# ska-telescope/ska-sdp-continuum-imaging-pipeline

Measured on AMD Instinct MI355X. Metric: Mvis/s gridded (invert) on 8k^2 grid, support=8, higher is better.
Workload: dtype f64; 1 GPU; C3: 390,625 rows x 256 ch = 100,000,000 vis/GPU -> 8192x8192 grid (4096^2 image), support 8, 2-D, fp64 accumulate; input=Stokes-I visibilities + effective weights (cip_ms2dirty), rows_per_gpu=390625, channels=256, grid=8192, image=4096, support=8, wstacking=False, parallelism=single GPU

## Files before the change

### ska-sdp-continuum-imaging-pipeline_amd/csrc/cip_grid.hip

```cpp
#include <type_traits>

#include "cip_internal.h"

namespace cip {


__global__ __launch_bounds__(1024) void prep_final_kernel(const double* partial, int nblocks, double* out2) {
  double sum[4] = {0.0, 0.0, 0.0, 0.0}, mx = 0.0;
  for (int i0 = threadIdx.x; i0 < nblocks; i0 += 4 * 1024) {
    if (i0 + 3 * 1024 < nblocks) {
      double2 p[4];
#pragma unroll
      for (int k = 0; k < 4; ++k) p[k] = reinterpret_cast<const double2*>(partial)[i0 + k * 1024];
#pragma unroll
      for (int k = 0; k < 4; ++k) {
        sum[k] += p[k].x;
        mx = fmax(mx, p[k].y);
      }
      continue;
    }
#pragma unroll
    for (int k = 0; k < 4; ++k) {
      const int i = i0 + k * 1024;
      if (i < nblocks) {
        const double2 p = reinterpret_cast<const double2*>(partial)[i];
        sum[k] += p.x;
        mx = fmax(mx, p.y);
      }
    }
  }
  double s = (sum[0] + sum[1]) + (sum[2] + sum[3]);
  for (int d = 32; d > 0; d >>= 1) {
    s += __shfl_xor(s, d, 64);
    mx = fmax(mx, __shfl_xor(mx, d, 64));
  }
  __shared__ double ss[16], sm[16];
  if ((threadIdx.x & 63) == 0) {
    ss[threadIdx.x >> 6] = s;
    sm[threadIdx.x >> 6] = mx;
  }
  __syncthreads();
  if (threadIdx.x == 0) {
    double t = 0.0, m = 0.0;
    for (int w = 0; w < 16; ++w) {
      t += ss[w];
      m = fmax(m, sm[w]);
    }
    out2[0] = t;
    out2[1] = m;
  }
}

hipError_t launch_prep_final(const double* partial, int nblocks, double* out2, hipStream_t s) {
  prep_final_kernel<<<dim3(1), dim3(1024), 0, s>>>(partial, nblocks, out2);
  return hipGetLastError();
}

__global__ void add_scalar_kernel(const double* src, double* dst) {
  if (threadIdx.x == 0) *dst += *src;
}

hipError_t launch_add_scalar(const double* src, double* dst, hipStream_t s) {
  add_scalar_kernel<<<dim3(1), dim3(64), 0, s>>>(src, dst);
  return hipGetLastError();
}

constexpr int kOrderThreads = 256;
constexpr int kOrderPer = kOrderWindow / kOrderThreads;
constexpr int kOrderBatch = kOrderThreads * kOrderPer;
static_assert(kOrderBatch == kOrderWindow, "one order block per window");

template <int WIDE, bool PH, int NC = 16>
__global__ __launch_bounds__(kOrderThreads, 8) void order_kernel(const uint8_t* __restrict__ vis_class, RowMap m,
                                                                 const uint64_t* __restrict__ runs,
                                                                 const int64_t* __restrict__ run_goff,
                                                                 const Chunk* __restrict__ windows,
                                                                 void* __restrict__ perm, int dP) {
  __shared__ __attribute__((aligned(16))) unsigned s_cnt[32];
  __shared__ unsigned s_keep[PH ? NC : 1], s_eff[PH ? NC : 1];
  __shared__ union {
    struct {
      uint64_t rec[kOrderBatch];
      int64_t delta[WIDE == 1 ? kOrderBatch : 1];
      int off[kOrderBatch + 1];
      uint16_t idx[kOrderBatch];
    } a;
    struct {
      unsigned S[kOrderBatch], M[kOrderBatch];
    } b;
  } sh;
  uint64_t* const s_rec = sh.a.rec;
  int* const s_off = sh.a.off;
  uint16_t* const s_idx = sh.a.idx;
  unsigned* const s_S = sh.b.S;
  unsigned* const s_M = sh.b.M;
  const Chunk ch = windows[blockIdx.x];
  const int64_t sb = ch.g0;
  const int nsb = (int)(ch.g1 - ch.g0);
  const int nst = (int)(ch.last_run - ch.first_run + 1);
  for (int k = threadIdx.x; k < nst; k += kOrderThreads) {
    s_off[k] = (int)(run_goff[ch.first_run + k] - sb);
    const uint64_t rec = runs[ch.first_run + k];
    if constexpr (WIDE == 2) {
      if (m.pk_runs) {
        s_rec[k] = rec;
      } else {
        const int64_t row = (int64_t)(rec >> 32), c = (int64_t)((rec >> 16) & 0xffff);
// ... 301 lines not shown
```

### ska-sdp-continuum-imaging-pipeline_amd/csrc/cip_internal.h

```cpp
#pragma once
#include <hip/hip_runtime.h>
#include <stdint.h>

#include <string>

#include "cip.h"
#include "cip_common.h"

namespace cip {

int set_error(int code, const std::string& msg);
#define CIP_HIP_CHECK(expr)                                                     \
  do {                                                                          \
    hipError_t e_ = (expr);                                                     \
    if (e_ != hipSuccess)                                                       \
      return ::cip::set_error(CIP_EHIP, std::string(#expr) + ": " +            \
                                            hipGetErrorString(e_));            \
  } while (0)

bool place_rows64();
bool order_classes32();

int64_t scan_tmp_elems(int64_t n);
hipError_t scan_run_offsets(const uint64_t* runs, int64_t nruns, int64_t* run_goff, int64_t* tmp,
                            const uint32_t* run_keys, hipStream_t s);
hipError_t exclusive_scan_i64(int64_t* data, int64_t n, int64_t* tmp, hipStream_t s);

hipError_t launch_freq_scale(const double* freq, int64_t nchan, double* fx, unsigned* err, hipStream_t s);
hipError_t launch_w_range(const double* uvw, int64_t nrow, double fxmin, double fxmax, double* partial,
                          int nblocks, hipStream_t s);
int plan_place_blocks(int64_t nvis);
hipError_t launch_prep_reduce(const RowMap& m, const void* vis, int vis_dtype, const void* wgt, int wgt_dtype,
                              const GridGeometry& g, unsigned* err_flag, double* partial, hipStream_t s);
hipError_t launch_plan_place(const double* uvw, const double* fx, const RowMap& m,
                             const void* vis, int vis_dtype, const void* wgt, int wgt_dtype, const GridGeometry& g,
                             unsigned* err_flag, uint8_t* vis_class, int64_t* blk_cnt, uint32_t* park_key,
                             uint64_t* park_run, double* partial, int64_t* hist0, hipStream_t s);
hipError_t launch_ragged_lengths(const int32_t* c0, const int32_t* c1, int64_t nrow, int64_t nchan, int64_t* out,
                                 unsigned* err, hipStream_t s);
hipError_t launch_ragged_expand(const int64_t* off, const int32_t* c0, int64_t nrow, int64_t* delta,
                                uint32_t* seg_row, hipStream_t s);
int64_t radix_blocks(int64_t n);
hipError_t launch_radix_hist(const uint32_t* keys, int64_t n, const int64_t* blk_cnt, int64_t nsub, int G, int shift,
                             int64_t* hist, hipStream_t s);
hipError_t launch_radix_group_hist(const int64_t* hist0, int64_t nsub, int G, int64_t* hg, hipStream_t s);
hipError_t launch_radix_scatter(const uint32_t* keys, const uint64_t* vals, int64_t n, const int64_t* blk_cnt,
                                int64_t nsub, int G, int shift, const int64_t* hist, uint32_t* keys_out,
                                uint64_t* vals_out, hipStream_t s);
hipError_t launch_tile_offsets(const uint32_t* keys, int64_t nruns, int64_t ntiles, int64_t* tile_run_off,
                               uint32_t kmask, hipStream_t s);
hipError_t launch_dirty_mask(const int64_t* tile_vis, const GridGeometry& g, uint8_t* mask, uint32_t* bits,
                             hipStream_t s);
hipError_t launch_tile_vis(const int64_t* run_goff, const int64_t* tile_run_off, int64_t ntiles,
                           int64_t* tile_vis_off, int64_t* tile_vis, hipStream_t s);
hipError_t launch_chunk_counts(const int64_t* tile_vis, int64_t ntiles, int64_t chunk_vis, int full_first,
                               int64_t* out, hipStream_t s);
hipError_t launch_chunk_emit(const int64_t* tile_vis_off, const int64_t* tile_vis, const int64_t* chunk_off,
                             const int64_t* run_goff, const int64_t* tile_run_off, int64_t ntiles,
                             int64_t chunk_vis, int full_first, int64_t nchunks, Chunk* chunks, hipStream_t s);
hipError_t launch_plane_chunk_counts(const int64_t* tile_vis_off, int64_t ntxy, int64_t ntw, int64_t ngroups,
                                     int group, int support, int64_t cv, int64_t* out, hipStream_t s);
hipError_t launch_plane_chunk_emit(const int64_t* tile_vis_off, const int64_t* chunk_off, const int64_t* run_goff,
                                   const int64_t* tile_run_off, int64_t ntxy, int64_t ntw, int64_t ngroups,
                                   int group, int support, int64_t cv, int64_t nchunks, Chunk* chunks, hipStream_t s);
hipError_t launch_gather_i64(const int64_t* src, int64_t stride, int64_t count, int64_t* dst,
                             hipStream_t s);

hipError_t launch_add_scalar(const double* src, double* dst, hipStream_t s);
hipError_t launch_prep_final(const double* partial, int nblocks, double* out2, hipStream_t s);
struct PlanView {
  const double *uvw = nullptr, *fx = nullptr;
  const void *vis = nullptr, *wgt = nullptr;
  RowMap m;
  const uint64_t* runs = nullptr;
  const int64_t *run_goff = nullptr, *tile_run_off = nullptr;
  const void* perm = nullptr;
  const Chunk* chunks = nullptr;
};
struct ScatterLaunch {
  PlanView plan;
  int64_t chunk_begin = 0, nchunks = 0;
  GridGeometry g;
  int64_t plane = 0;
  double fixed_scale = 1.0;
  double* grid = nullptr;
  int support = 0, vis_dtype = CIP_C64, wgt_dtype = CIP_NONE;
  bool packed = false;
  int group = 1;
  bool share_cus = false, store_private = false;
};
template <int W>
hipError_t launch_scatter_w(const ScatterLaunch& a, dim3 gd, unsigned lds_extra, hipStream_t s);
template <int W>
hipError_t launch_scatter_large_w(const ScatterLaunch& a, dim3 gd, hipStream_t s);
hipError_t launch_scatter(const ScatterLaunch& a, hipStream_t s);
hipError_t launch_order(const uint8_t* vis_class, const RowMap& m, const uint64_t* runs, const int64_t* run_goff,
                        const Chunk* windows, int64_t nwindows, void* perm, int phase_support, hipStream_t s);
bool order_phases_ok(const RowMap& m, int support);
hipError_t launch_crop_correct_2d(const double* grid, const GridGeometry& g, int64_t npix_x, int64_t npix_y,
                                  const double* cx, const double* cy, double* dirty, hipStream_t s);
hipError_t launch_wplane_accumulate(const double* grid, const GridGeometry& g, int64_t npix_x, int64_t npix_y,
                                    double pixsize_x, double pixsize_y, double w_plane, int first,
                                    double* acc, hipStream_t s);
hipError_t launch_wfinal_correct(double* acc, int64_t npix_x, int64_t npix_y, double pixsize_x, double pixsize_y,
                                 const double* cx, const double* cy, const double* fw_table, int64_t fw_n,
                                 double fw_dnu, double dw, int64_t i0, int64_t nrows, const double* norm,
                                 const float* acc_f32, hipStream_t s);

struct DegridOut {
  void* vis_io;
  int vis_dtype;
  const void* wgt;
  int wgt_dtype;
  int subtract;
  double2* acc;
};
struct DegridLaunch {
  PlanView plan;
  int64_t chunk_begin = 0, nchunks = 0;
  GridGeometry g;
  int64_t plane = 0;
  const double* planes = nullptr;
// ... 75 lines not shown
```

### ska-sdp-continuum-imaging-pipeline_amd/csrc/cip_plan.hip

```cpp
#include <type_traits>

#include "cip_internal.h"

namespace cip {

constexpr int kScanThreads = 1024;
constexpr int kScanItems = 4;
constexpr int64_t kScanBlock = (int64_t)kScanThreads * kScanItems;

template <int RUNS>
__device__ __forceinline__ int64_t run_length_at(const void* __restrict__ src, int64_t k) {
  if constexpr (RUNS == 2) {
    return (int64_t)(((const uint32_t*)src)[k] >> kRunLenShift) + 1;
  } else {
    const uint64_t rec = ((const uint64_t*)src)[k];
    return (int64_t)(rec & 0xffff) - (int64_t)((rec >> 16) & 0xffff);
  }
}
template <int RUNS>
__global__ __launch_bounds__(kScanThreads) void scan_local_kernel(int64_t* data, int64_t n, int64_t* block_sums,
                                                                  const void* __restrict__ runs) {
  __shared__ int64_t wave_tot[kScanThreads / 64];
  const int64_t base = (int64_t)blockIdx.x * kScanBlock + (int64_t)threadIdx.x * kScanItems;
  int64_t v[kScanItems];
  int64_t tsum = 0;
  if (base + kScanItems <= (RUNS ? n - 1 : n)) {
#pragma unroll
    for (int i = 0; i < kScanItems; ++i) {
      if constexpr (RUNS) {
        v[i] = run_length_at<RUNS>(runs, base + i);
      } else {
        v[i] = data[base + i];
      }
    }
  } else {
#pragma unroll
    for (int i = 0; i < kScanItems; ++i) {
      if constexpr (RUNS) {
        v[i] = 0;
        if (base + i < n - 1) v[i] = run_length_at<RUNS>(runs, base + i);
      } else {
        v[i] = (base + i < n) ? data[base + i] : 0;
      }
    }
  }
#pragma unroll
  for (int i = 0; i < kScanItems; ++i) tsum += v[i];
  const int lane = threadIdx.x & 63, wave = threadIdx.x >> 6;
  int64_t incl = tsum;
#pragma unroll
  for (int d = 1; d < 64; d <<= 1) {
    int64_t o = __shfl_up(incl, d, 64);
    if (lane >= d) incl += o;
  }
  if (lane == 63) wave_tot[wave] = incl;
  __syncthreads();
  if (wave == 0) {
    int64_t t = (lane < kScanThreads / 64) ? wave_tot[lane] : 0;
#pragma unroll
    for (int d = 1; d < 64; d <<= 1) {
      int64_t o = __shfl_up(t, d, 64);
      if (lane >= d) t += o;
    }
    if (lane < kScanThreads / 64) wave_tot[lane] = t;
  }
  __syncthreads();
  int64_t run = incl - tsum + (wave > 0 ? wave_tot[wave - 1] : 0);
#pragma unroll
  for (int i = 0; i < kScanItems; ++i) {
    if (base + i < n) data[base + i] = run;
    run += v[i];
  }
  if (threadIdx.x == kScanThreads - 1) block_sums[blockIdx.x] = run;
}

__global__ void scan_add_kernel(int64_t* data, int64_t n, const int64_t* offsets) {
  const int64_t i = (int64_t)blockIdx.x * kScanBlock + threadIdx.x;
  const int64_t off = offsets[blockIdx.x];
  if (i + (int64_t)(kScanItems - 1) * kScanThreads < n) {
    int64_t v[kScanItems];
#pragma unroll
    for (int k = 0; k < kScanItems; ++k) v[k] = data[i + (int64_t)k * kScanThreads];
#pragma unroll
    for (int k = 0; k < kScanItems; ++k) data[i + (int64_t)k * kScanThreads] = v[k] + off;
    return;
  }
#pragma unroll
  for (int k = 0; k < kScanItems; ++k) {
    const int64_t j = i + (int64_t)k * kScanThreads;
    if (j < n) data[j] += off;
  }
}

int64_t scan_tmp_elems(int64_t n) {
  int64_t total = 0;
  while (n > 1) {
    const int64_t nb = (n + kScanBlock - 1) / kScanBlock;
    total += nb;
    n = nb;
  }
  return total + 1;
}

struct ScanLengths {
  int kind;
  const void* src;
};
static hipError_t scan_impl(int64_t* data, int64_t n, int64_t* tmp, ScanLengths from, hipStream_t s) {
  if (n <= 0) return hipSuccess;
  const int64_t nb = (n + kScanBlock - 1) / kScanBlock;
  hipError_t e = dispatch_int<0, 1, 2>(from.kind, hipErrorInvalidValue, [&](auto kind) {
    scan_local_kernel<decltype(kind)::value><<<dim3((unsigned)nb), dim3(kScanThreads), 0, s>>>(data, n, tmp, from.src);
    return hipGetLastError();
  });
  if (e != hipSuccess || nb == 1) return e;
  e = scan_impl(tmp, nb, tmp + nb, ScanLengths{0, nullptr}, s);
  if (e != hipSuccess) return e;
  scan_add_kernel<<<dim3((unsigned)nb), dim3(kScanThreads), 0, s>>>(data, n, tmp);
  return hipGetLastError();
}

hipError_t exclusive_scan_i64(int64_t* data, int64_t n, int64_t* tmp, hipStream_t s) {
  return scan_impl(data, n, tmp, ScanLengths{0, nullptr}, s);
}

hipError_t scan_run_offsets(const uint64_t* runs, int64_t nruns, int64_t* run_goff, int64_t* tmp,
                            const uint32_t* run_keys, hipStream_t s) {
  return scan_impl(run_goff, nruns + 1, tmp, run_keys ? ScanLengths{2, run_keys} : ScanLengths{1, runs}, s);
}

__global__ void freq_scale_kernel(const double* freq, int64_t nchan, double* fx, unsigned* err) {
  const int64_t c = (int64_t)blockIdx.x * blockDim.x + threadIdx.x;
  if (c < nchan) {
    const double f = freq[c];
    fx[c] = f / CIP_SPEED_OF_LIGHT;
    if (err && !(f > 0.0 && isfinite(f))) atomicOr(err, 4u);
  }
}

hipError_t launch_freq_scale(const double* freq, int64_t nchan, double* fx, unsigned* err, hipStream_t s) {
  freq_scale_kernel<<<dim3((unsigned)((nchan + 255) / 256)), dim3(256), 0, s>>>(freq, nchan, fx, err);
  return hipGetLastError();
}

__global__ __launch_bounds__(256) void w_range_kernel(const double* uvw, int64_t nrow, double fxmin, double fxmax,
                                                      double* partial) {
  double lo = INFINITY, hi = -INFINITY;
  for (int64_t r = (int64_t)blockIdx.x * 256 + threadIdx.x; r < nrow; r += (int64_t)gridDim.x * 256) {
    const double w = uvw[3 * r + 2];
    const double a = w * fxmin, b = w * fxmax;
    lo = fmin(lo, fmin(a, b));
    hi = fmax(hi, fmax(a, b));
  }
  for (int d = 32; d > 0; d >>= 1) {
    lo = fmin(lo, __shfl_xor(lo, d, 64));
    hi = fmax(hi, __shfl_xor(hi, d, 64));
  }
  __shared__ double sl[4], sh[4];
  if ((threadIdx.x & 63) == 0) { sl[threadIdx.x >> 6] = lo; sh[threadIdx.x >> 6] = hi; }
  __syncthreads();
  if (threadIdx.x == 0) {
    for (int i = 1; i < 4; ++i) { lo = fmin(lo, sl[i]); hi = fmax(hi, sh[i]); }
    partial[2 * blockIdx.x] = lo;
    partial[2 * blockIdx.x + 1] = hi;
  }
}

hipError_t launch_w_range(const double* uvw, int64_t nrow, double fxmin, double fxmax, double* partial,
                          int nblocks, hipStream_t s) {
  w_range_kernel<<<dim3(nblocks), dim3(256), 0, s>>>(uvw, nrow, fxmin, fxmax, partial);
  return hipGetLastError();
// ... 378 lines not shown
      return hipGetLastError();
    });
  });
}

__global__ void ragged_lengths_kernel(const int32_t* __restrict__ c0, const int32_t* __restrict__ c1, int64_t nrow,
                                      int64_t nchan, int64_t* __restrict__ out, unsigned* err) {
  const int64_t r = (int64_t)blockIdx.x * blockDim.x + threadIdx.x;
  if (r < nrow) {
    const int32_t a = c0[r], b = c1[r];
    const bool ok = a >= 0 && a <= b && (int64_t)b <= nchan;
    if (!ok) atomicOr(err, 1u);
    out[r] = ok ? (int64_t)(b - a) : 0;
  } else if (r == nrow) {
    out[r] = 0;
  }
}

hipError_t launch_ragged_lengths(const int32_t* c0, const int32_t* c1, int64_t nrow, int64_t nchan, int64_t* out,
                                 unsigned* err, hipStream_t s) {
  ragged_lengths_kernel<<<dim3((unsigned)((nrow + 256) / 256)), dim3(256), 0, s>>>(c0, c1, nrow, nchan, out, err);
  return hipGetLastError();
}

__global__ __launch_bounds__(256) void ragged_expand_kernel(const int64_t* __restrict__ off,
                                                            const int32_t* __restrict__ c0, int64_t nrow,
                                                            int64_t* __restrict__ delta,
                                                            uint32_t* __restrict__ seg_row) {
  const int64_t r = (int64_t)blockIdx.x * blockDim.x + threadIdx.x;
  if (r >= nrow) return;
  const int64_t a = off[r], b = off[r + 1];
  delta[r] = a - (int64_t)c0[r];
  for (int64_t k = (a + 63) >> 6; k * 64 < b; ++k) seg_row[k] = (uint32_t)r;
}

hipError_t launch_ragged_expand(const int64_t* off, const int32_t* c0, int64_t nrow, int64_t* delta,
                                uint32_t* seg_row, hipStream_t s) {
  if (nrow <= 0) return hipSuccess;
  ragged_expand_kernel<<<dim3((unsigned)((nrow + 255) / 256)), dim3(256), 0, s>>>(off, c0, nrow, delta, seg_row);
  return hipGetLastError();
}

constexpr int kRadixThreads = 256;
constexpr int kRadixPer = 16;
constexpr int64_t kRadixBlock = (int64_t)kRadixThreads * kRadixPer;
static_assert(kRadixBlock == 64 * 64, "a radix sub-block covers one place block's park region");

__device__ __forceinline__ int64_t radix_count(int64_t b, int64_t n, const int64_t* __restrict__ blk_cnt) {
  if (blk_cnt) return blk_cnt[b];
  const int64_t rem = n - b * kRadixBlock;
  return rem < kRadixBlock ? rem : kRadixBlock;
}

__global__ __launch_bounds__(kRadixThreads) void radix_hist_kernel(const uint32_t* __restrict__ keys, int64_t n,
                                                                   const int64_t* __restrict__ blk_cnt, int64_t nsub,
                                                                   int G, int shift, int64_t ngroups,
                                                                   int64_t* __restrict__ hist) {
  __shared__ unsigned cnt[256];
  cnt[threadIdx.x] = 0u;
  __syncthreads();
  const int64_t b0 = (int64_t)blockIdx.x * G;
  const int64_t b1 = b0 + G < nsub ? b0 + G : nsub;
  for (int64_t b = b0; b < b1; ++b) {
    const int64_t cnt_b = radix_count(b, n, blk_cnt);
    const uint32_t* kb = keys + b * kRadixBlock;
    if (cnt_b == kRadixBlock) {
      uint32_t kk[kRadixPer];
#pragma unroll
      for (int k = 0; k < kRadixPer; ++k) kk[k] = kb[threadIdx.x + k * kRadixThreads];
#pragma unroll
      for (int k = 0; k < kRadixPer; ++k) atomicAdd(&cnt[(kk[k] >> shift) & 255u], 1u);
    } else {
      for (int64_t i = threadIdx.x; i < cnt_b; i += kRadixThreads) atomicAdd(&cnt[(kb[i] >> shift) & 255u], 1u);
    }
  }
  __syncthreads();
  hist[(int64_t)threadIdx.x * ngroups + blockIdx.x] = cnt[threadIdx.x];
  if (blockIdx.x == 0 && threadIdx.x == 0) hist[256 * ngroups] = 0;
}

__global__ void radix_group_hist_kernel(const int64_t* __restrict__ hist0, int64_t nsub, int G, int64_t ngroups,
                                        int64_t* __restrict__ hg) {
  const int64_t t = (int64_t)blockIdx.x * blockDim.x + threadIdx.x;
  if (t == 0) hg[256 * ngroups] = 0;
  if (t >= 256 * ngroups) return;
  const int64_t d = t / ngroups, gi = t - d * ngroups;
  const int64_t b0 = gi * G, b1 = b0 + G < nsub ? b0 + G : nsub;
  int64_t sum = 0;
  for (int64_t b = b0; b < b1; ++b) sum += hist0[d * nsub + b];
  hg[t] = sum;
}

__global__ __launch_bounds__(kRadixThreads) void radix_scatter_kernel(
    const uint32_t* __restrict__ keys, const uint64_t* __restrict__ vals, int64_t n,
    const int64_t* __restrict__ blk_cnt, int64_t nsub, int G, int shift, int64_t ngroups,
    const int64_t* __restrict__ hist, uint32_t* __restrict__ keys_out, uint64_t* __restrict__ vals_out) {
  __shared__ unsigned wcnt[4][256];
  __shared__ int64_t dnext[256];
  __shared__ int64_t woff[4][256];
  const int lane = threadIdx.x & 63, wave = threadIdx.x >> 6;
  dnext[threadIdx.x] = hist[(int64_t)threadIdx.x * ngroups + blockIdx.x];
  const int64_t b0 = (int64_t)blockIdx.x * G;
  const int64_t b1 = b0 + G < nsub ? b0 + G : nsub;
  for (int64_t b = b0; b < b1; ++b) {
    const int64_t cnt_b = radix_count(b, n, blk_cnt);
    const int steps = (int)((cnt_b + 255) / 256);
    const int q = 64 * steps;
    const int64_t i0 = b * kRadixBlock + wave * q + lane;
    const int64_t wlim = b * kRadixBlock + (int64_t)(wave + 1) * q;
    const int64_t blim = b * kRadixBlock + cnt_b;
    const int64_t lim = wlim < blim ? wlim : blim;
#pragma unroll
    for (int w = 0; w < 4; ++w) wcnt[w][threadIdx.x] = 0u;
    uint32_t key[kRadixPer];
    uint64_t val[kRadixPer];
#pragma unroll
    for (int k = 0; k < kRadixPer; ++k) {
      const int64_t i = i0 + k * 64;
      key[k] = (k < steps && i < lim) ? keys[i] : 0u;
      val[k] = (k < steps && i < lim) ? vals[i] : 0ull;
    }
    __syncthreads();
    unsigned rank[kRadixPer];
#pragma unroll
    for (int k = 0; k < kRadixPer; ++k) {
      if (k < steps) {
        const bool valid = i0 + k * 64 < lim;
        const unsigned d = (key[k] >> shift) & 255u;
        unsigned long long peers = __ballot(valid);
#pragma unroll
        for (int bit = 0; bit < 8; ++bit) {
          const bool on = (d >> bit) & 1u;
          const unsigned long long m = __ballot(on);
          peers &= on ? m : ~m;
        }
        const unsigned prior = valid ? wcnt[wave][d] : 0u;
        rank[k] = prior + (unsigned)__popcll(peers & ((1ull << lane) - 1ull));
        if (valid && (peers & ((1ull << lane) - 1ull)) == 0ull) wcnt[wave][d] = prior + (unsigned)__popcll(peers);
      }
    }
    __syncthreads();
    {
      const int d = threadIdx.x;
      int64_t o = dnext[d];
#pragma unroll
      for (int w = 0; w < 4; ++w) {
        woff[w][d] = o;
        o += wcnt[w][d];
      }
      dnext[d] = o;
    }
    __syncthreads();
#pragma unroll
    for (int k = 0; k < kRadixPer; ++k)
      if (k < steps && i0 + k * 64 < lim) {
        const int64_t pos = woff[wave][(key[k] >> shift) & 255u] + rank[k];
        keys_out[pos] = key[k];
        vals_out[pos] = val[k];
      }
    __syncthreads();
  }
}

__global__ void tile_offsets_kernel(const uint32_t* __restrict__ keys, int64_t nruns, int64_t ntiles,
                                    int64_t* __restrict__ tile_run_off, uint32_t kmask) {
  const int64_t t = (int64_t)blockIdx.x * blockDim.x + threadIdx.x;
  if (t > ntiles) return;
  int64_t lo = 0, hi = nruns;
  while (lo < hi) {
    const int64_t mid = (lo + hi) >> 1;
    if ((int64_t)(keys[mid] & kmask) < t) lo = mid + 1;
    else hi = mid;
  }
  tile_run_off[t] = lo;
}

int64_t radix_blocks(int64_t n) { return (n + kRadixBlock - 1) / kRadixBlock; }

hipError_t launch_radix_hist(const uint32_t* keys, int64_t n, const int64_t* blk_cnt, int64_t nsub, int G, int shift,
                             int64_t* hist, hipStream_t s) {
  if (nsub == 0) return hipSuccess;
  const int64_t ngroups = (nsub + G - 1) / G;
  radix_hist_kernel<<<dim3((unsigned)ngroups), dim3(kRadixThreads), 0, s>>>(keys, n, blk_cnt, nsub, G, shift,
                                                                          ngroups, hist);
  return hipGetLastError();
}

hipError_t launch_radix_group_hist(const int64_t* hist0, int64_t nsub, int G, int64_t* hg, hipStream_t s) {
  const int64_t ngroups = (nsub + G - 1) / G;
  const int64_t nt = 256 * ngroups > 0 ? 256 * ngroups : 1;
  radix_group_hist_kernel<<<dim3((unsigned)((nt + 255) / 256)), dim3(256), 0, s>>>(hist0, nsub, G, ngroups, hg);
  return hipGetLastError();
}

hipError_t launch_radix_scatter(const uint32_t* keys, const uint64_t* vals, int64_t n, const int64_t* blk_cnt,
                                int64_t nsub, int G, int shift, const int64_t* hist, uint32_t* keys_out,
                                uint64_t* vals_out, hipStream_t s) {
  if (nsub == 0) return hipSuccess;
  const int64_t ngroups = (nsub + G - 1) / G;
  radix_scatter_kernel<<<dim3((unsigned)ngroups), dim3(kRadixThreads), 0, s>>>(
      keys, vals, n, blk_cnt, nsub, G, shift, ngroups, hist, keys_out, vals_out);
  return hipGetLastError();
}

hipError_t launch_tile_offsets(const uint32_t* keys, int64_t nruns, int64_t ntiles, int64_t* tile_run_off,
                               uint32_t kmask, hipStream_t s) {
  tile_offsets_kernel<<<dim3((unsigned)((ntiles + 256) / 256)), dim3(256), 0, s>>>(keys, nruns, ntiles, tile_run_off,
                                                                                 kmask);
  return hipGetLastError();
}

__global__ void tile_vis_kernel(const int64_t* run_goff, const int64_t* tile_run_off, int64_t ntiles,
                                int64_t* tile_vis_off, int64_t* tile_vis) {
  const int64_t t = (int64_t)blockIdx.x * blockDim.x + threadIdx.x;
  if (t > ntiles) return;
  const int64_t a = run_goff[tile_run_off[t]];
  tile_vis_off[t] = a;
  if (t < ntiles) tile_vis[t] = run_goff[tile_run_off[t + 1]] - a;
}

__global__ void dirty_mask_kernel(const int64_t* __restrict__ tile_vis, GridGeometry g, uint8_t* __restrict__ mask) {
  const int64_t ntx = g.ntx, nty = g.nty, ntw = g.ntw, nplanes = g.nplanes;
  const int support = g.support;
  const int64_t id = (int64_t)blockIdx.x * blockDim.x + threadIdx.x;
  const int64_t nt = ntx * nty;
  if (id >= nt * nplanes) return;
  const int64_t p = id / nt, t = id - p * nt;
  int64_t lo = 0, hi = 0;
  if (nplanes > 1) {
    lo = p - support + 1 > 0 ? p - support + 1 : 0;
    hi = p < ntw - 1 ? p : ntw - 1;
  }
  bool touched = false;
  for (int64_t w = lo; w <= hi && !touched; ++w) touched = tile_vis[t * ntw + w] > 0;
  if (!touched) return;
  uint8_t* m = mask + p * g.mtx * g.mty;
  const int64_t mx0 = (t % ntx) << (g.tx_shift - kTileShift), my0 = (t / ntx) << (g.ty_shift - kTileShift);
// ... 212 lines not shown
```

### ska-sdp-continuum-imaging-pipeline_amd/csrc/cip_planner.hip

```cpp
#include <algorithm>
#include <cmath>
#include <cstring>

#include "cip_host.h"

namespace cip {

static int64_t chunk_vis(bool packed, int64_t nu) {
  return packed ? kChunkVisPacked : (nu >= 16384 ? kChunkVis / 2 : kChunkVis);
}

static int radix_group(int pass) { return pass ? 1 : 8; }

static bool wgt_dtype_ok(int d) { return d == CIP_NONE || d == CIP_F32 || d == CIP_F64 || d == CIP_POL4I; }

static int plan_error(unsigned errbits) {
  if (errbits & 4u) return set_error(CIP_EINVAL, "channel frequencies must be positive");
  if (errbits & 2u) return set_error(CIP_EINVAL, "non-finite visibility or weight");
  if (errbits & 1u)
    return set_error(CIP_ERANGE, "non-finite (u, v, w) coordinates, or w outside the w-plane stack");
  return CIP_OK;
}

static int make_plan(Workspace* ws, const double* uvw, const double* fx, const RowMap& m,
                     const void* vis, int vis_dtype, const void* wgt, int wgt_dtype, double* red,
                     const GridGeometry& g, int64_t cv, hipStream_t s, PlanResult* pr, double* maxabs,
                     int group = 1) {
  const int64_t ntiles = g.ntx * g.nty * g.ntw;
  pr->ntiles = ntiles;
  pr->phases = false;
  CIP_ALLOC(tile_runs, int64_t, "tile_runs", ntiles + 1)
  CIP_ALLOC(tile_vis, int64_t, "tile_vis", ntiles + 1)
  CIP_ALLOC(tile_vis_off, int64_t, "tile_vis_off", ntiles + 1)
  CIP_ALLOC(chunk_off, int64_t, "chunk_off", 2 * ntiles + 1)
  CIP_ALLOC(err, unsigned, "err_flag", 1)
  CIP_ALLOC(scan_tmp, int64_t, "scan_tmp", scan_tmp_elems(ntiles + 1))
  const int64_t nvis = m.nvis;
  const int nblk = plan_place_blocks(nvis);
  const bool ragged = m.delta != nullptr;
  const bool order = scatter_order() && (ragged || nvis < ((int64_t)1 << 32));
  uint8_t* vis_class = nullptr;
  if (order) {
    vis_class = buf<uint8_t>(ws, "vis_class", nvis);
    if (!vis_class) return CIP_ENOMEM;
  }
  CIP_ALLOC(blk_cnt, int64_t, "blk_cnt", nblk)
  CIP_ALLOC(park_key, uint32_t, "park_key", (int64_t)nblk * 4096)
  CIP_ALLOC(park_run, uint64_t, "park_run", (int64_t)nblk * 4096)
  CIP_ALLOC(partial, double, "prep_partial", 2 * nblk)
  const int g0 = radix_group(0), g1 = radix_group(1);
  const int64_t ng0 = (nblk + g0 - 1) / g0;
  CIP_ALLOC(hist0, int64_t, "radix_hist0", 256 * (int64_t)nblk + 1)
  CIP_ALLOC(hist0g, int64_t, "radix_hist0g", 256 * ng0 + 1)
  CIP_ALLOC(scan_h0, int64_t, "scan_hist0", scan_tmp_elems(256 * ng0 + 1))
  int key_bits = 1;
  while (key_bits < 32 && ((int64_t)1 << key_bits) < ntiles) ++key_bits;
  const int npass = (key_bits + 7) / 8;
  RowMap mp = m;
  mp.pk_runs = (ragged && m.pk_cbits && order && g.support <= 16 && 8 * npass <= kRunLenShift && packed_runs()) ? 1 : 0;
  CIP_HIP_CHECK(launch_plan_place(uvw, fx, mp, vis, vis_dtype, wgt, wgt_dtype, g, err, vis_class, blk_cnt, park_key,
                                  park_run, partial, hist0, s));
  CIP_HIP_CHECK(launch_prep_final(partial, nblk, red, s));
  CIP_HIP_CHECK(launch_radix_group_hist(hist0, nblk, g0, hist0g, s));
  CIP_HIP_CHECK(exclusive_scan_i64(hist0g, 256 * ng0 + 1, scan_h0, s));
  int64_t* h = (int64_t*)pinned(ws, 4 * sizeof(int64_t));
  if (!h) return CIP_ENOMEM;
  CIP_HIP_CHECK(hipMemcpyAsync(&h[0], hist0g + 256 * ng0, sizeof(int64_t), hipMemcpyDeviceToHost, s));
  CIP_HIP_CHECK(hipMemcpyAsync(&h[1], err, sizeof(unsigned), hipMemcpyDeviceToHost, s));
  CIP_HIP_CHECK(hipMemcpyAsync(&h[2], red + 1, sizeof(double), hipMemcpyDeviceToHost, s));
  CIP_HIP_CHECK(hipStreamSynchronize(s));
  const int64_t nruns = h[0];
  std::memcpy(maxabs, &h[2], sizeof(double));
  if (const int rc = plan_error((unsigned)h[1]); rc != CIP_OK) return rc;
  pr->nruns = nruns;
  CIP_ALLOC(key_a, uint32_t, "sort_key_a", nruns)
  CIP_ALLOC(key_b, uint32_t, "sort_key_b", nruns)
  CIP_ALLOC(run_a, uint64_t, "sort_run_a", nruns)
  CIP_ALLOC(run_b, uint64_t, "sort_run_b", nruns)
  const int64_t nbd = radix_blocks(nruns);
  const int64_t ng1 = (nbd + g1 - 1) / g1;
  CIP_ALLOC(hist, int64_t, "radix_hist", 256 * ng1 + 1)
  CIP_ALLOC(scan_h, int64_t, "scan_hist", scan_tmp_elems(256 * ng1 + 1))
  CIP_HIP_CHECK(launch_radix_scatter(park_key, park_run, 0, blk_cnt, nblk, g0, 0, hist0g, key_a, run_a, s));
  uint32_t *kin = key_a, *kout = key_b;
  uint64_t *rin = run_a, *rout = run_b;
  for (int p = 1; p < npass; ++p) {
    CIP_HIP_CHECK(launch_radix_hist(kin, nruns, nullptr, nbd, g1, 8 * p, hist, s));
    CIP_HIP_CHECK(exclusive_scan_i64(hist, 256 * ng1 + 1, scan_h, s));
    CIP_HIP_CHECK(launch_radix_scatter(kin, rin, nruns, nullptr, nbd, g1, 8 * p, hist, kout, rout, s));
    std::swap(kin, kout);
    std::swap(rin, rout);
  }
  uint64_t* runs = rin;
  CIP_HIP_CHECK(launch_tile_offsets(kin, nruns, ntiles, tile_runs, mp.pk_runs ? kRunKeyMask : 0xffffffffu, s));
  const int64_t* tile_run_off = tile_runs;
  CIP_ALLOC(run_goff, int64_t, "run_goff", nruns + 1)
  CIP_ALLOC(scan_tmp2, int64_t, "scan_tmp2", scan_tmp_elems(nruns + 1))
  CIP_HIP_CHECK(scan_run_offsets(runs, nruns, run_goff, scan_tmp2, mp.pk_runs ? kin : nullptr, s));
  CIP_HIP_CHECK(launch_tile_vis(run_goff, tile_run_off, ntiles, tile_vis_off, tile_vis, s));
  if (g.mtx % 32 == 0 && grid_mask()) {
    CIP_ALLOC(dmask, uint8_t, "dirty_mask", g.mtx * g.mty * g.nplanes)
    CIP_ALLOC(dbits, uint32_t, "dirty_bits", g.mtx * g.mty / 32 * g.nplanes + (g.mty + 31) / 32 * g.nplanes)
// ... 164 lines not shown
    const int rc = choose(rq.npix_x, rq.npix_y, rq.px, rq.py, rq.epsilon, rq.support, rq.do_wstacking, wmin, wmax,
                          &out->p);
    if (rc != CIP_OK) return rc;
  }
  const bool tile_ok = rq.wide_tile && !ragged && scatter_order() && m.nvis < ((int64_t)1 << 32);
  TileShape shape = scatter_tile_shape(out->p, packed, tile_ok);
  const TileShape saved_shape{ws->saved_plan.tx_shift, ws->saved_plan.ty_shift};
  const bool saved32 = saved_shape.tx_shift == kTileShift && saved_shape.ty_shift == kTileShift;
  const bool reusing =
      reusable && ((saved_shape.tx_shift == shape.tx_shift && saved_shape.ty_shift == shape.ty_shift) || saved32);
  if (reusing) shape = saved_shape;
  out->g = geometry(out->p, rq.px, rq.py, shape);
  if (rq.plane_end >= 0) {
    if (rq.plane_begin < 0 || rq.plane_begin > rq.plane_end || rq.plane_end > out->p.nplanes)
      return set_error(CIP_EINVAL, "w-plane range outside [0, nplanes]");
    out->g.plane_lo = rq.plane_begin;
    out->g.plane_hi = rq.plane_end;
  }
  if ((double)out->g.ntx * (double)out->g.nty * (double)out->g.ntw >= 4294967295.0)
    return set_error(CIP_EINVAL, "grid tiles x w layers exceed the 32-bit tile key space");
  if (packed && vis_dtype != CIP_C64 && vis_dtype != CIP_POL4I)
    return set_error(CIP_EINVAL, "single-precision accumulation needs complex64 visibilities");
  if (packed && out->g.support > 16)
    return set_error(CIP_EINVAL, "single-precision accumulation supports kernel supports <= 16");
  out->packed = packed;
  out->fixed_scale = 1.0;
  out->fx = fx;
  out->red = red;
  const int group = rq.want_group ? wstack_group(out->g, packed) : 1;
  if (grid_out) {
    const int64_t gplanes = group;
    const bool f32 = packed && grid_is_transposed(out->g, rq.npix_x, rq.npix_y) && grid_f32_enabled();
    const size_t gbytes = (f32 ? sizeof(float) : sizeof(double)) * 2 * out->g.nu * out->g.nv * gplanes;
    double* grid = buf<double>(ws, "grid", 2 * out->g.nu * out->g.nv * gplanes);
    if (!grid) return CIP_ENOMEM;
    if (ws->grid_clean != grid || ws->grid_clean_bytes < gbytes) {
      const int zr = zero_on_side(ws, grid, gbytes, s);
      if (zr != CIP_OK) return zr;
    }
    *grid_out = grid;
  }
  hipEvent_t e_prep = g_prof.mark(s);
  g_prof.span(0, g_prof.pool.empty() ? nullptr : g_prof.pool[0], e_prep);
  if (nrow == 0 || m.nvis == 0) {
    CIP_HIP_CHECK(hipMemsetAsync(red, 0, 2 * sizeof(double), s));
    out->plan = PlanResult();
    out->plan.plane_chunk_off.assign((out->g.do_wstacking ? out->g.nplanes : 1) + 1, 0);
    return CIP_OK;
  }
  double maxabs = 0.0;
  int rc;
  if (reusing) {
    const int nblk = plan_place_blocks(m.nvis);
    CIP_ALLOC(partial, double, "prep_partial_reuse", 2 * nblk)
    CIP_HIP_CHECK(launch_prep_reduce(m, rq.vis, vis_dtype, rq.wgt, wgt_dtype, out->g, err, partial, s));
    CIP_HIP_CHECK(launch_prep_final(partial, nblk, red, s));
    unsigned* h = (unsigned*)pinned(ws, 4 * sizeof(double));
    if (!h) return CIP_ENOMEM;
    CIP_HIP_CHECK(hipMemcpyAsync(h, err, sizeof(unsigned), hipMemcpyDeviceToHost, s));
    CIP_HIP_CHECK(hipMemcpyAsync((double*)h + 1, red + 1, sizeof(double), hipMemcpyDeviceToHost, s));
    CIP_HIP_CHECK(hipStreamSynchronize(s));
    std::memcpy(&maxabs, (double*)h + 1, sizeof(double));
    if (rc = plan_error(h[0]); rc != CIP_OK) return rc;
    out->plan = ws->saved_plan;
  } else {
    ws->saved_valid = false;
    rc = make_plan(ws, rq.uvw, fx, m, rq.vis, vis_dtype, rq.wgt, wgt_dtype, red, out->g, chunk_vis(packed, out->g.nu),
                   s, &out->plan, &maxabs, group);
    out->plan.tx_shift = out->g.tx_shift;
    out->plan.ty_shift = out->g.ty_shift;
    if (rc == CIP_OK && !ragged) {
      ws->saved_key = key;
      ws->saved_p = out->p;
      ws->saved_plan = out->plan;
      ws->saved_valid = true;
    }
  }
  g_prof.span(1, e_prep, g_prof.mark(s));
  if (rc != CIP_OK) return rc;
  if (!std::isfinite(maxabs)) return set_error(CIP_EINVAL, "non-finite visibility or weight");
  int e2 = 0;
  if (maxabs > 0.0) std::frexp(maxabs, &e2);
  out->fixed_scale = std::ldexp(1.0, (packed ? kPackedBits : kFixedBits) - e2);
  g_prof.counts[0] = m.nvis;
  g_prof.counts[1] = out->plan.nruns;
  g_prof.counts[2] = out->plan.nchunks;
  g_prof.counts[3] = out->g.nplanes;
  return rc;
}

}
```

Measured before the change: 23340 Mvis/s.

## Use wave-sized blocks with DPP scans and ballot histograms in planning kernels

The single-block prep reduction is split into sixteen 64-thread blocks that each write a per-wave total, followed by a tiny final kernel. The prefix scan now runs one wave per 4096-item block, scanning in rounds with DPP lane shifts and a carry instead of shared memory and barriers. The radix histogram swaps LDS atomics for ballot/popcount counting in 64-thread blocks. The aim is to cut barrier and atomic overhead in the planning stage, at the cost of less parallelism per block and an extra kernel launch.

After: 23870 Mvis/s (median of 6 runs). 2.3% higher.

```diff
diff --git a/ska-sdp-continuum-imaging-pipeline_amd/csrc/cip_grid.hip b/ska-sdp-continuum-imaging-pipeline_amd/csrc/cip_grid.hip
--- a/ska-sdp-continuum-imaging-pipeline_amd/csrc/cip_grid.hip
+++ b/ska-sdp-continuum-imaging-pipeline_amd/csrc/cip_grid.hip
@@ -5,25 +5,37 @@
 namespace cip {
 
 
-__global__ __launch_bounds__(1024) void prep_final_kernel(const double* partial, int nblocks, double* out2) {
-  double sum[4] = {0.0, 0.0, 0.0, 0.0}, mx = 0.0;
-  for (int i0 = threadIdx.x; i0 < nblocks; i0 += 4 * 1024) {
-    if (i0 + 3 * 1024 < nblocks) {
-      double2 p[4];
-#pragma unroll
-      for (int k = 0; k < 4; ++k) p[k] = reinterpret_cast<const double2*>(partial)[i0 + k * 1024];
-#pragma unroll
-      for (int k = 0; k < 4; ++k) {
-        sum[k] += p[k].x;
-        mx = fmax(mx, p[k].y);
-      }
-      continue;
-    }
-#pragma unroll
-    for (int k = 0; k < 4; ++k) {
-      const int i = i0 + k * 1024;
+constexpr int kPrepWaves = 16, kPrepAcc = 4;
+constexpr int kPrepThreads = 64 * kPrepWaves;
+constexpr int kPrepStride = kPrepAcc * kPrepThreads;
+constexpr int kPrepUnroll = 4;
+static_assert(2 * kPrepWaves <= kPrepFinalScratch, "a {sum, max} pair per wave behind the partials");
+
+__global__ __launch_bounds__(64) void prep_wave_totals_kernel(const double* partial, int nblocks, double* totals) {
+  const double2* p2 = reinterpret_cast<const double2*>(partial);
+  double sum[kPrepAcc] = {0.0, 0.0, 0.0, 0.0}, mx = 0.0;
+  int i0 = (int)blockIdx.x * 64 + (int)threadIdx.x;
+  for (; (int64_t)i0 + (kPrepUnroll - 1) * kPrepStride + (kPrepAcc - 1) * kPrepThreads < nblocks;
+       i0 += kPrepUnroll * kPrepStride) {
+    double2 p[kPrepUnroll][kPrepAcc];
+#pragma unroll
+    for (int j = 0; j < kPrepUnroll; ++j)
+#pragma unroll
+      for (int k = 0; k < kPrepAcc; ++k) p[j][k] = p2[i0 + j * kPrepStride + k * kPrepThreads];
+#pragma unroll
+    for (int j = 0; j < kPrepUnroll; ++j)
+#pragma unroll
+      for (int k = 0; k < kPrepAcc; ++k) {
+        sum[k] += p[j][k].x;
+        mx = fmax(mx, p[j][k].y);
+      }
+  }
+  for (; i0 < nblocks; i0 += kPrepStride) {
+#pragma unroll
+    for (int k = 0; k < kPrepAcc; ++k) {
+      const int64_t i = (int64_t)i0 + k * kPrepThreads;
       if (i < nblocks) {
-        const double2 p = reinterpret_cast<const double2*>(partial)[i];
+        const double2 p = p2[i];
         sum[k] += p.x;
         mx = fmax(mx, p.y);
       }
@@ -34,25 +46,27 @@
     s += __shfl_xor(s, d, 64);
     mx = fmax(mx, __shfl_xor(mx, d, 64));
   }
-  __shared__ double ss[16], sm[16];
-  if ((threadIdx.x & 63) == 0) {
-    ss[threadIdx.x >> 6] = s;
-    sm[threadIdx.x >> 6] = mx;
-  }
-  __syncthreads();
   if (threadIdx.x == 0) {
-    double t = 0.0, m = 0.0;
-    for (int w = 0; w < 16; ++w) {
-      t += ss[w];
-      m = fmax(m, sm[w]);
-    }
-    out2[0] = t;
-    out2[1] = m;
-  }
-}
-
-hipError_t launch_prep_final(const double* partial, int nblocks, double* out2, hipStream_t s) {
-  prep_final_kernel<<<dim3(1), dim3(1024), 0, s>>>(partial, nblocks, out2);
+    totals[2 * blockIdx.x] = s;
+    totals[2 * blockIdx.x + 1] = mx;
+  }
+}
+
+__global__ __launch_bounds__(64) void prep_final_kernel(const double* totals, double* out2) {
+  if (threadIdx.x != 0) return;
+  double t = 0.0, m = 0.0;
+  for (int w = 0; w < kPrepWaves; ++w) {
+    t += totals[2 * w];
+    m = fmax(m, totals[2 * w + 1]);
+  }
+  out2[0] = t;
+  out2[1] = m;
+}
+
+hipError_t launch_prep_final(double* partial, int nblocks, double* out2, hipStream_t s) {
+  double* totals = partial + 2 * (int64_t)nblocks;
+  prep_wave_totals_kernel<<<dim3(kPrepWaves), dim3(64), 0, s>>>(partial, nblocks, totals);
+  prep_final_kernel<<<dim3(1), dim3(64), 0, s>>>(totals, out2);
   return hipGetLastError();
 }
 
diff --git a/ska-sdp-continuum-imaging-pipeline_amd/csrc/cip_internal.h b/ska-sdp-continuum-imaging-pipeline_amd/csrc/cip_internal.h
--- a/ska-sdp-continuum-imaging-pipeline_amd/csrc/cip_internal.h
+++ b/ska-sdp-continuum-imaging-pipeline_amd/csrc/cip_internal.h
@@ -66,8 +66,9 @@
 hipError_t launch_gather_i64(const int64_t* src, int64_t stride, int64_t count, int64_t* dst,
                              hipStream_t s);
 
+constexpr int kPrepFinalScratch = 32;
 hipError_t launch_add_scalar(const double* src, double* dst, hipStream_t s);
-hipError_t launch_prep_final(const double* partial, int nblocks, double* out2, hipStream_t s);
+hipError_t launch_prep_final(double* partial, int nblocks, double* out2, hipStream_t s);
 struct PlanView {
   const double *uvw = nullptr, *fx = nullptr;
   const void *vis = nullptr, *wgt = nullptr;
diff --git a/ska-sdp-continuum-imaging-pipeline_amd/csrc/cip_plan.hip b/ska-sdp-continuum-imaging-pipeline_amd/csrc/cip_plan.hip
--- a/ska-sdp-continuum-imaging-pipeline_amd/csrc/cip_plan.hip
+++ b/ska-sdp-continuum-imaging-pipeline_amd/csrc/cip_plan.hip
@@ -4,9 +4,36 @@
 
 namespace cip {
 
-constexpr int kScanThreads = 1024;
+constexpr int kScanThreads = 64;
 constexpr int kScanItems = 4;
-constexpr int64_t kScanBlock = (int64_t)kScanThreads * kScanItems;
+constexpr int kScanRound = kScanThreads * kScanItems;
+constexpr int kScanRounds = 16;
+constexpr int kScanBatch = 4;
+constexpr int64_t kScanBlock = (int64_t)kScanRound * kScanRounds;
+static_assert(kScanBlock == 4096, "scan_tmp_elems and every caller's scratch size assume 4096 items per block");
+static_assert(kScanRounds % kScanBatch == 0, "whole batches");
+
+template <int CTRL, int ROW_MASK>
+__device__ __forceinline__ int64_t dpp_or_zero(int64_t v) {
+  const uint32_t lo = (uint32_t)__builtin_amdgcn_update_dpp(0, (int)(uint32_t)v, CTRL, ROW_MASK, 0xf, false);
+  const uint32_t hi =
+      (uint32_t)__builtin_amdgcn_update_dpp(0, (int)(uint32_t)((uint64_t)v >> 32), CTRL, ROW_MASK, 0xf, false);
+  return (int64_t)(((uint64_t)hi << 32) | (uint64_t)lo);
+}
+__device__ __forceinline__ int64_t wave_scan_incl(int64_t x) {
+  x += dpp_or_zero<0x111, 0xf>(x);
+  x += dpp_or_zero<0x112, 0xf>(x);
+  x += dpp_or_zero<0x114, 0xf>(x);
+  x += dpp_or_zero<0x118, 0xf>(x);
+  x += dpp_or_zero<0x142, 0xa>(x);
+  x += dpp_or_zero<0x143, 0xc>(x);
+  return x;
+}
+__device__ __forceinline__ int64_t read_lane63(int64_t v) {
+  const uint32_t lo = (uint32_t)__builtin_amdgcn_readlane((int)(uint32_t)v, 63);
+  const uint32_t hi = (uint32_t)__builtin_amdgcn_readlane((int)(uint32_t)((uint64_t)v >> 32), 63);
+  return (int64_t)(((uint64_t)hi << 32) | (uint64_t)lo);
+}
 
 template <int RUNS>
 __device__ __forceinline__ int64_t run_length_at(const void* __restrict__ src, int64_t k) {
@@ -17,77 +44,76 @@
     return (int64_t)(rec & 0xffff) - (int64_t)((rec >> 16) & 0xffff);
   }
 }
+template <int RUNS, bool FULL>
+__device__ __forceinline__ int64_t scan_rounds(int64_t* data, int64_t n, int64_t nin, const void* __restrict__ runs,
+                                               int64_t b0, int lane) {
+  int64_t carry = 0;
+#pragma unroll
+  for (int r0 = 0; r0 < kScanRounds; r0 += kScanBatch) {
+    if (!FULL && b0 + (int64_t)r0 * kScanRound >= n) break;
+    int64_t v[kScanBatch][kScanItems];
+#pragma unroll
+    for (int q = 0; q < kScanBatch; ++q) {
+      const int64_t base = b0 + (int64_t)(r0 + q) * kScanRound + (int64_t)lane * kScanItems;
+#pragma unroll
+      for (int i = 0; i < kScanItems; ++i) {
+        if constexpr (FULL) {
+          if constexpr (RUNS) v[q][i] = run_length_at<RUNS>(runs, base + i);
+          else v[q][i] = data[base + i];
+        } else {
+          v[q][i] = 0;
+          if (base + i < nin) {
+            if constexpr (RUNS) v[q][i] = run_length_at<RUNS>(runs, base + i);
+            else v[q][i] = data[base + i];
+          }
+        }
+      }
+    }
+#pragma unroll
+    for (int q = 0; q < kScanBatch; ++q) {
+      const int64_t base = b0 + (int64_t)(r0 + q) * kScanRound + (int64_t)lane * kScanItems;
+      int64_t tsum = 0;
+#pragma unroll
+      for (int i = 0; i < kScanItems; ++i) tsum += v[q][i];
+      const int64_t incl = wave_scan_incl(tsum);
+      int64_t run = carry + (incl - tsum);
+#pragma unroll
+      for (int i = 0; i < kScanItems; ++i) {
+        if (FULL || base + i < n) data[base + i] = run;
+        run += v[q][i];
+      }
+      carry += read_lane63(incl);
+    }
+  }
+  return carry;
+}
 template <int RUNS>
 __global__ __launch_bounds__(kScanThreads) void scan_local_kernel(int64_t* data, int64_t n, int64_t* block_sums,
                                                                   const void* __restrict__ runs) {
-  __shared__ int64_t wave_tot[kScanThreads / 64];
-  const int64_t base = (int64_t)blockIdx.x * kScanBlock + (int64_t)threadIdx.x * kScanItems;
-  int64_t v[kScanItems];
-  int64_t tsum = 0;
-  if (base + kScanItems <= (RUNS ? n - 1 : n)) {
-#pragma unroll
-    for (int i = 0; i < kScanItems; ++i) {
-      if constexpr (RUNS) {
-        v[i] = run_length_at<RUNS>(runs, base + i);
-      } else {
-        v[i] = data[base + i];
-      }
-    }
-  } else {
-#pragma unroll
-    for (int i = 0; i < kScanItems; ++i) {
-      if constexpr (RUNS) {
-        v[i] = 0;
-        if (base + i < n - 1) v[i] = run_length_at<RUNS>(runs, base + i);
-      } else {
-        v[i] = (base + i < n) ? data[base + i] : 0;
-      }
-    }
-  }
-#pragma unroll
-  for (int i = 0; i < kScanItems; ++i) tsum += v[i];
-  const int lane = threadIdx.x & 63, wave = threadIdx.x >> 6;
-  int64_t incl = tsum;
-#pragma unroll
-  for (int d = 1; d < 64; d <<= 1) {
-    int64_t o = __shfl_up(incl, d, 64);
-    if (lane >= d) incl += o;
-  }
-  if (lane == 63) wave_tot[wave] = incl;
-  __syncthreads();
-  if (wave == 0) {
-    int64_t t = (lane < kScanThreads / 64) ? wave_tot[lane] : 0;
-#pragma unroll
-    for (int d = 1; d < 64; d <<= 1) {
-      int64_t o = __shfl_up(t, d, 64);
-      if (lane >= d) t += o;
-    }
-    if (lane < kScanThreads / 64) wave_tot[lane] = t;
-  }
-  __syncthreads();
-  int64_t run = incl - tsum + (wave > 0 ? wave_tot[wave - 1] : 0);
-#pragma unroll
-  for (int i = 0; i < kScanItems; ++i) {
-    if (base + i < n) data[base + i] = run;
-    run += v[i];
-  }
-  if (threadIdx.x == kScanThreads - 1) block_sums[blockIdx.x] = run;
-}
-
-__global__ void scan_add_kernel(int64_t* data, int64_t n, const int64_t* offsets) {
+  const int lane = threadIdx.x;
+  const int64_t b0 = (int64_t)blockIdx.x * kScanBlock;
+  const int64_t nin = RUNS ? n - 1 : n;
+  const int64_t total = b0 + kScanBlock <= nin ? scan_rounds<RUNS, true>(data, n, nin, runs, b0, lane)
+                                               : scan_rounds<RUNS, false>(data, n, nin, runs, b0, lane);
+  if (lane == 0) block_sums[blockIdx.x] = total;
+}
+
+constexpr int kScanAddThreads = 256;
+constexpr int kScanAddItems = (int)(kScanBlock / kScanAddThreads);
+__global__ __launch_bounds__(kScanAddThreads) void scan_add_kernel(int64_t* data, int64_t n, const int64_t* offsets) {
   const int64_t i = (int64_t)blockIdx.x * kScanBlock + threadIdx.x;
   const int64_t off = offsets[blockIdx.x];
-  if (i + (int64_t)(kScanItems - 1) * kScanThreads < n) {
-    int64_t v[kScanItems];
-#pragma unroll
-    for (int k = 0; k < kScanItems; ++k) v[k] = data[i + (int64_t)k * kScanThreads];
-#pragma unroll
-    for (int k = 0; k < kScanItems; ++k) data[i + (int64_t)k * kScanThreads] = v[k] + off;
+  if ((int64_t)(blockIdx.x + 1) * kScanBlock <= n) {
+    int64_t v[kScanAddItems];
+#pragma unroll
+    for (int k = 0; k < kScanAddItems; ++k) v[k] = data[i + (int64_t)k * kScanAddThreads];
+#pragma unroll
+    for (int k = 0; k < kScanAddItems; ++k) data[i + (int64_t)k * kScanAddThreads] = v[k] + off;
     return;
   }
 #pragma unroll
-  for (int k = 0; k < kScanItems; ++k) {
-    const int64_t j = i + (int64_t)k * kScanThreads;
+  for (int k = 0; k < kScanAddItems; ++k) {
+    const int64_t j = i + (int64_t)k * kScanAddThreads;
     if (j < n) data[j] += off;
   }
 }
@@ -116,7 +142,7 @@
   if (e != hipSuccess || nb == 1) return e;
   e = scan_impl(tmp, nb, tmp + nb, ScanLengths{0, nullptr}, s);
   if (e != hipSuccess) return e;
-  scan_add_kernel<<<dim3((unsigned)nb), dim3(kScanThreads), 0, s>>>(data, n, tmp);
+  scan_add_kernel<<<dim3((unsigned)nb), dim3(kScanAddThreads), 0, s>>>(data, n, tmp);
   return hipGetLastError();
 }
 
@@ -601,31 +627,62 @@
   return rem < kRadixBlock ? rem : kRadixBlock;
 }
 
-__global__ __launch_bounds__(kRadixThreads) void radix_hist_kernel(const uint32_t* __restrict__ keys, int64_t n,
-                                                                   const int64_t* __restrict__ blk_cnt, int64_t nsub,
-                                                                   int G, int shift, int64_t ngroups,
-                                                                   int64_t* __restrict__ hist) {
-  __shared__ unsigned cnt[256];
-  cnt[threadIdx.x] = 0u;
-  __syncthreads();
+constexpr int kRadixHistThreads = 64;
+constexpr int kRadixHistBatch = 16;
+static_assert(kRadixBlock % (64 * kRadixHistBatch) == 0, "whole batches in a full sub-block");
+
+__device__ __forceinline__ void radix_hist_step(uint32_t digit, bool valid, const uint32_t (&flip)[6],
+                                                unsigned (&cnt)[4]) {
+  unsigned long long m[8];
+#pragma unroll
+  for (int b = 0; b < 8; ++b) m[b] = __ballot((digit >> b) & 1u);
+  const unsigned long long vm = __ballot(valid);
+  uint32_t lo = 0xffffffffu, hi = 0xffffffffu;
+#pragma unroll
+  for (int b = 0; b < 6; ++b) {
+    lo &= (uint32_t)m[b] ^ flip[b];
+    hi &= (uint32_t)(m[b] >> 32) ^ flip[b];
+  }
+#pragma unroll
+  for (int q = 0; q < 4; ++q) {
+    const unsigned long long sel = vm & ((q & 1) ? m[6] : ~m[6]) & ((q & 2) ? m[7] : ~m[7]);
+    cnt[q] += (unsigned)__popc(lo & (uint32_t)sel) + (unsigned)__popc(hi & (uint32_t)(sel >> 32));
+  }
+}
+
+__global__ __launch_bounds__(kRadixHistThreads) void radix_hist_kernel(const uint32_t* __restrict__ keys, int64_t n,
+                                                                       const int64_t* __restrict__ blk_cnt,
+                                                                       int64_t nsub, int G, int shift,
+                                                                       int64_t ngroups, int64_t* __restrict__ hist) {
+  const int lane = threadIdx.x;
+  uint32_t flip[6];
+#pragma unroll
+  for (int b = 0; b < 6; ++b) flip[b] = ((lane >> b) & 1) ? 0u : 0xffffffffu;
+  unsigned cnt[4] = {0u, 0u, 0u, 0u};
   const int64_t b0 = (int64_t)blockIdx.x * G;
   const int64_t b1 = b0 + G < nsub ? b0 + G : nsub;
   for (int64_t b = b0; b < b1; ++b) {
-    const int64_t cnt_b = radix_count(b, n, blk_cnt);
+    const int cnt_b = (int)radix_count(b, n, blk_cnt);
     const uint32_t* kb = keys + b * kRadixBlock;
-    if (cnt_b == kRadixBlock) {
-      uint32_t kk[kRadixPer];
-#pragma unroll
-      for (int k = 0; k < kRadixPer; ++k) kk[k] = kb[threadIdx.x + k * kRadixThreads];
-#pragma unroll
-      for (int k = 0; k < kRadixPer; ++k) atomicAdd(&cnt[(kk[k] >> shift) & 255u], 1u);
-    } else {
-      for (int64_t i = threadIdx.x; i < cnt_b; i += kRadixThreads) atomicAdd(&cnt[(kb[i] >> shift) & 255u], 1u);
-    }
-  }
-  __syncthreads();
-  hist[(int64_t)threadIdx.x * ngroups + blockIdx.x] = cnt[threadIdx.x];
-  if (blockIdx.x == 0 && threadIdx.x == 0) hist[256 * ngroups] = 0;
+    for (int i0 = 0; i0 < cnt_b; i0 += 64 * kRadixHistBatch) {
+      uint32_t kk[kRadixHistBatch];
+      if (i0 + 64 * kRadixHistBatch <= cnt_b) {
+#pragma unroll
+        for (int k = 0; k < kRadixHistBatch; ++k) kk[k] = kb[i0 + 64 * k + lane];
+#pragma unroll
+        for (int k = 0; k < kRadixHistBatch; ++k) radix_hist_step((kk[k] >> shift) & 255u, true, flip, cnt);
+      } else {
+        for (int i = i0; i < cnt_b; i += 64) {
+          const bool valid = i + lane < cnt_b;
+          const uint32_t key = valid ? kb[i + lane] : 0u;
+          radix_hist_step((key >> shift) & 255u, valid, flip, cnt);
+        }
+      }
+    }
+  }
+#pragma unroll
+  for (int q = 0; q < 4; ++q) hist[(int64_t)(lane + 64 * q) * ngroups + blockIdx.x] = cnt[q];
+  if (blockIdx.x == 0 && lane == 0) hist[256 * ngroups] = 0;
 }
 
 __global__ void radix_group_hist_kernel(const int64_t* __restrict__ hist0, int64_t nsub, int G, int64_t ngroups,
@@ -730,8 +787,8 @@
                              int64_t* hist, hipStream_t s) {
   if (nsub == 0) return hipSuccess;
   const int64_t ngroups = (nsub + G - 1) / G;
-  radix_hist_kernel<<<dim3((unsigned)ngroups), dim3(kRadixThreads), 0, s>>>(keys, n, blk_cnt, nsub, G, shift,
-                                                                          ngroups, hist);
+  radix_hist_kernel<<<dim3((unsigned)ngroups), dim3(kRadixHistThreads), 0, s>>>(keys, n, blk_cnt, nsub, G, shift,
+                                                                              ngroups, hist);
   return hipGetLastError();
 }
 
diff --git a/ska-sdp-continuum-imaging-pipeline_amd/csrc/cip_planner.hip b/ska-sdp-continuum-imaging-pipeline_amd/csrc/cip_planner.hip
--- a/ska-sdp-continuum-imaging-pipeline_amd/csrc/cip_planner.hip
+++ b/ska-sdp-continuum-imaging-pipeline_amd/csrc/cip_planner.hip
@@ -47,7 +47,7 @@
   CIP_ALLOC(blk_cnt, int64_t, "blk_cnt", nblk)
   CIP_ALLOC(park_key, uint32_t, "park_key", (int64_t)nblk * 4096)
   CIP_ALLOC(park_run, uint64_t, "park_run", (int64_t)nblk * 4096)
-  CIP_ALLOC(partial, double, "prep_partial", 2 * nblk)
+  CIP_ALLOC(partial, double, "prep_partial", 2 * nblk + kPrepFinalScratch)
   const int g0 = radix_group(0), g1 = radix_group(1);
   const int64_t ng0 = (nblk + g0 - 1) / g0;
   CIP_ALLOC(hist0, int64_t, "radix_hist0", 256 * (int64_t)nblk + 1)
@@ -318,7 +318,7 @@
   int rc;
   if (reusing) {
     const int nblk = plan_place_blocks(m.nvis);
-    CIP_ALLOC(partial, double, "prep_partial_reuse", 2 * nblk)
+    CIP_ALLOC(partial, double, "prep_partial_reuse", 2 * nblk + kPrepFinalScratch)
     CIP_HIP_CHECK(launch_prep_reduce(m, rq.vis, vis_dtype, rq.wgt, wgt_dtype, out->g, err, partial, s));
     CIP_HIP_CHECK(launch_prep_final(partial, nblk, red, s));
     unsigned* h = (unsigned*)pinned(ws, 4 * sizeof(double));
```
